# zhiqwang/yolort

Hardware: AMD Instinct MI355X
Metric: images/sec at 640x640 (bs=32) yolov5s (higher is better)
Workload: dtype fp16; 1 GPU; yolov5_darknet_pan_s_r60 fp16 bs=32/GPU 640x640 fixed-size stream (letterbox = identity: the stem reads the planar images) -> backbone+PAN+head+decode+NMS HIP path (BASELINE configs[1]); detections_per_img=300, weights=seeded synthetic (workloads/synth.py, head_gain 0.4), parallelism=dp1 (one shard per rank, slab all-gather), conv_tiles=pinned table yolort_amd/data/tiles_gfx950.json

## Files before the change

yolort_amd/csrc/stem_body1_fused.hip:

```cpp
#include "conv_common.hpp"

namespace ymi {

constexpr int SB_TH = 8, SB_TW = 16;
constexpr int SB_PH = 2 * SB_TH + 1, SB_PW = 2 * SB_TW + 1;
constexpr int SB_NE = SB_TW + 1;
constexpr int SB_PPIX = SB_PH * SB_PW;
constexpr int SB_GROUPS = (SB_PPIX + 31) / 32;
constexpr int SB_IR = 2 * SB_PH + 4, SB_IC = 80;
constexpr int SB_ENTRIES = 3 * SB_IR * (SB_IC / 8);
constexpr int SB_PIECES = (SB_ENTRIES + 63) / 64;
constexpr int SB_SW = SB_PW + 2;
constexpr int SB_SENTRIES = SB_IR * SB_SW;
constexpr int SB_SPIECES = (SB_SENTRIES + 63) / 64;
constexpr int SB_MAX_IMGS = 32;
#ifndef YMI_SB_PK
#define YMI_SB_PK 0
#endif
constexpr bool SB_PK = YMI_SB_PK != 0;

struct SbImgs {
    const uint16_t* img[SB_MAX_IMGS];
};

constexpr int SB_W1 = 0, SB_W2 = 36 * 1024, SB_B2 = 256, SB_PLANAR = SB_SPIECES * 1024, SB_PATCH = ((SB_PPIX + 15) / 16) * 1024;
constexpr int SB_LDS = SB_W1 + SB_W2 + SB_B2 + SB_PLANAR + SB_PATCH;

template <int DT, bool PLANAR>
__global__ __launch_bounds__(512, 1) void stem_body1_fused_kernel(const ConvArgs a1, const ConvArgs a2, const SbImgs pl, int tiles_x, int tiles_y, int ntiles) {
    typedef typename Mfma<DT>::frag frag;
    extern __shared__ __attribute__((aligned(16))) unsigned char sb_sm[];
    frag* w2l = reinterpret_cast<frag*>(sb_sm + SB_W1);
    f32x4* b2l = reinterpret_cast<f32x4*>(sb_sm + SB_W1 + SB_W2);
    uint16_t* planar = reinterpret_cast<uint16_t*>(sb_sm + SB_W1 + SB_W2 + SB_B2);
    unsigned char* patch = sb_sm + SB_W1 + SB_W2 + SB_B2 + SB_PLANAR;

    const int tid = threadIdx.x;
    const int lane = tid & 63;
    const int wave = __builtin_amdgcn_readfirstlane(tid >> 6);
    const int hi = lane >> 5, px = lane & 31;
    const int H = a1.h, W = 2 * a1.w_in;

    {
        for (int f = wave; f < 36; f += 8) {
            const int i = f & 1, ts = f >> 1;
            w2l[f * 64 + lane] = *reinterpret_cast<const frag*>(a2.w + (int64_t)(i * 32 + px) * a2.k_pad + ts * 16 + hi * 8);
        }
        if (tid < 16) {
            const int t = tid >> 3, g = (tid >> 1) & 3, h = tid & 1;
            b2l[tid] = *reinterpret_cast<const f32x4*>(a2.bias + t * 32 + g * 8 + h * 4);
        }
    }
    f32x4 bias1[1][4];
    load_bias<1>(a1, 0, hi, bias1);
    frag wf1[9];
    {
        const uint16_t* wr = a1.w + (int64_t)px * a1.k_pad + 8 * hi;
#pragma unroll
        for (int s = 0; s < 9; ++s) wf1[s] = *reinterpret_cast<const frag*>(wr + 16 * s);
    }

    int e_plane[3], e_row[3], e_col[3];
#pragma unroll
    for (int j = 0; j < 3; ++j) {
        const int e = (wave * 3 + j) * 64 + lane;
        if constexpr (PLANAR) {
            const int ec = e < SB_ENTRIES ? e : SB_ENTRIES - 1;
            const int plane = ec / (SB_IR * (SB_IC / 8));
            const int rem = ec - plane * (SB_IR * (SB_IC / 8));
            const int pr = rem / (SB_IC / 8), seg = rem - pr * (SB_IC / 8);
            e_plane[j] = e < SB_ENTRIES ? plane : -1;
            e_row[j] = pr - 4;
            e_col[j] = 8 * seg - 8;
        } else {
            const int ec = e < SB_SENTRIES ? e : SB_SENTRIES - 1;
            const int pr = ec / SB_SW, sc = ec - pr * SB_SW;
            e_plane[j] = e < SB_SENTRIES ? 0 : -1;
            e_row[j] = pr - 4;
            e_col[j] = sc - 2;
        }
    }
    auto tile_origin = [&](int idx, int& img, int& oy0, int& ox0) {
        int t = xcd_remap(idx, ntiles);
        const int tx = t % tiles_x;
        t /= tiles_x;
        const int ty = t % tiles_y;
        img = t / tiles_y;
        oy0 = ty * SB_TH;
        ox0 = tx * SB_TW;
    };
    auto issue_planar = [&](int idx) {
        int img, oy0, ox0;
        tile_origin(idx, img, oy0, ox0);
        if constexpr (PLANAR) {
            const uint16_t* base = pl.img[img];
#pragma unroll
            for (int j = 0; j < 3; ++j) {
                const int pi = wave * 3 + j;
                if (pi < SB_PIECES) {
                    const int iy = 4 * oy0 + e_row[j], ix = 4 * ox0 + e_col[j];
                    const bool ok = (e_plane[j] >= 0) && ((unsigned)iy < (unsigned)H) && ((unsigned)ix < (unsigned)W);
                    const uint16_t* src = ok ? base + ((int64_t)e_plane[j] * H + iy) * W + ix : a1.zeros;
                    glds16(src, planar + pi * 512);
                }
            }
        } else {
#pragma unroll
            for (int j = 0; j < 3; ++j) {
                const int pi = wave * 3 + j;
                if (pi < SB_SPIECES) {
                    const int iy = 4 * oy0 + e_row[j], isp = 2 * ox0 + e_col[j];
                    const bool ok = (e_plane[j] >= 0) && ((unsigned)iy < (unsigned)H) && ((unsigned)isp < (unsigned)a1.w_in);
                    const uint16_t* src = ok ? a1.x + ((int64_t)(img * H + iy) * a1.w_in + isp) * a1.x_cs : a1.zeros;
                    glds16(src, planar + pi * 512);
                }
            }
        }
    };

    int s1_off[3], s1_rc[3], s1_dst[3];
#pragma unroll
    for (int j = 0; j < 3; ++j) {
        const int g = wave + 8 * j;
        const int q = g * 32 + px;
        const int qc = q < SB_PPIX ? q : SB_PPIX - 1;
        const int pr = qc / SB_PW, rem = qc - pr * SB_PW;
        const int pc = rem < SB_NE ? 2 * rem : 2 * (rem - SB_NE) + 1;
        s1_rc[j] = q < SB_PPIX ? ((pr << 16) | pc) : -1;
        s1_off[j] = PLANAR ? (2 * pr) * SB_IC + 2 * pc + 4
                           : ((2 * pr) * SB_SW + pc) * 8;
        s1_dst[j] = qc * 64 + ((hi ^ ((qc >> 2) & 3)) * 16);
    }
    const int pg = wave & 3, ct = wave >> 2;
    const int pr_o = (pg * 32 + px) / SB_TW, pc_o = (pg * 32 + px) % SB_TW;
    int ea[9];
#pragma unroll
    for (int t = 0; t < 9; ++t) {
        const int dy = t / 3, dx = t % 3;
        const int col = 2 * pc_o + dx;
        const int slot = (col & 1) ? SB_NE + (col >> 1) : (col >> 1);
        const int q = (2 * pr_o + dy) * SB_PW + slot;
        ea[t] = (q * 32 + ((hi ^ ((q >> 2) & 3)) * 8)) * 2;
    }
    constexpr int PLANE_HALFS = SB_IR * SB_IC;

    int idx = blockIdx.x;
    if (idx < ntiles) issue_planar(idx);
    for (; idx < ntiles; idx += gridDim.x) {
        int img, oy0, ox0;
        tile_origin(idx, img, oy0, ox0);
        asm volatile("s_waitcnt vmcnt(0)" ::: "memory");
        __syncthreads();

#pragma unroll
        for (int j = 0; j < 3; ++j) {
            if (wave + 8 * j < SB_GROUPS) {
                f32x16 acc[1][1];
                init_acc<1, 1>(acc, bias1);
                if constexpr (PLANAR) {
                    uint32_t rr[9], gg[9], bb[9];
#pragma unroll
                    for (int s = 0; s < 9; ++s) {
                        const int tap0 = 2 * s, tap1 = 2 * s + 1;
                        const int o0 = (tap0 / 3) * SB_IC + 2 * (tap0 % 3), o1 = (tap1 / 3) * SB_IC + 2 * (tap1 % 3);
                        const uint16_t* p0 = planar + s1_off[j] + (hi ? o1 : o0);
                        rr[s] = *reinterpret_cast<const uint32_t*>(p0);
                        gg[s] = *reinterpret_cast<const uint32_t*>(p0 + PLANE_HALFS);
                        bb[s] = *reinterpret_cast<const uint32_t*>(p0 + 2 * PLANE_HALFS);
                    }
                    __builtin_amdgcn_sched_barrier(0);
#pragma unroll
                    for (int s = 0; s < 9; ++s) {
                        const uint32_t r = rr[s], g = gg[s], b = bb[s];
                        u32x4 q;
                        q[0] = (r & 0xffffu) | (g << 16);
                        q[1] = b & 0xffffu;
                        q[2] = (r >> 16) | (g & 0xffff0000u);
                        q[3] = b >> 16;
                        frag af;
                        __builtin_memcpy(&af, &q, 16);
                        acc[0][0] = Mfma<DT>::run(wf1[s], af, acc[0][0]);
                    }
                } else {
                    frag af[9];
#pragma unroll
                    for (int s = 0; s < 9; ++s) {
                        const int tap0 = 2 * s, tap1 = 2 * s + 1;
                        const int o0 = ((tap0 / 3) * SB_SW + (tap0 % 3)) * 8, o1 = ((tap1 / 3) * SB_SW + (tap1 % 3)) * 8;
                        af[s] = *reinterpret_cast<const frag*>(planar + s1_off[j] + (hi ? o1 : o0));
                    }
                    __builtin_amdgcn_sched_barrier(0);
#pragma unroll
                    for (int s = 0; s < 9; ++s) acc[0][0] = Mfma<DT>::run(wf1[s], af[s], acc[0][0]);
                }
                const u32x2 norv[4] = {};
                u32x4 o[2];
                silu_pack_subtile<DT, false, true, SB_PK>(acc[0][0], norv, o);
                const int sy = 2 * oy0 - 1 + (s1_rc[j] >> 16), sx = 2 * ox0 - 1 + (s1_rc[j] & 0xffff);
                const bool in = s1_rc[j] >= 0 && ((unsigned)sy < (unsigned)a1.ho) && ((unsigned)sx < (unsigned)a1.wo);
                if (!in) {
                    o[0] = u32x4{0u, 0u, 0u, 0u};
                    o[1] = u32x4{0u, 0u, 0u, 0u};
                }
                if (s1_rc[j] >= 0) {
                    *reinterpret_cast<u32x4*>(patch + s1_dst[j]) = o[0];
                    *reinterpret_cast<u32x4*>(patch + (s1_dst[j] ^ 32)) = o[1];
                }
            }
        }
        __syncthreads();
        if (idx + (int)gridDim.x < ntiles) issue_planar(idx + gridDim.x);

        f32x16 acc2[1][1];
#pragma unroll
        for (int g = 0; g < 4; ++g) {
            const f32x4 b = b2l[(ct * 4 + g) * 2 + hi];
#pragma unroll
            for (int e = 0; e < 4; ++e) acc2[0][0][g * 4 + e] = b[e];
        }
#pragma unroll
        for (int half = 0; half < 2; ++half) {
            frag fa[9], fw[9];
#pragma unroll
            for (int u = 0; u < 9; ++u) {
                const int ts = half * 9 + u;
                fa[u] = *reinterpret_cast<const frag*>(patch + ((ts & 1) ? (ea[ts >> 1] ^ 32) : ea[ts >> 1]));
                fw[u] = w2l[(ts * 2 + ct) * 64 + lane];
            }
            __builtin_amdgcn_sched_barrier(0);
#pragma unroll
            for (int u = 0; u < 9; ++u) acc2[0][0] = Mfma<DT>::run(fw[u], fa[u], acc2[0][0]);
        }
        finish_wave_tile<DT, DT, 1, 1>(a2, acc2, ct * 32, hi, [&](int, int64_t& m, bool& ok) {
            const int oy = oy0 + pr_o, ox = ox0 + pc_o;
            ok = oy < a2.ho && ox < a2.wo;
            m = ((int64_t)img * a2.ho + oy) * a2.wo + ox;
        });
    }
}

template <int DT, bool PLANAR>
static int stem_body1_launch_t(const ConvArgs& s0, const ConvArgs& b0, const void* const* imgs, hipStream_t st) {
    const int tiles_x = cdiv(b0.wo, SB_TW), tiles_y = cdiv(b0.ho, SB_TH);
    auto kfn = stem_body1_fused_kernel<DT, PLANAR>;
    { const int rc_lds = allow_big_lds((const void*)kfn, SB_LDS); if (rc_lds != YMI_OK) return rc_lds; }
    const int per_launch = PLANAR ? SB_MAX_IMGS : b0.n;
    for (int base = 0; base < b0.n; base += per_launch) {
        ConvArgs a1 = s0, a2 = b0;
        const int n = b0.n - base < per_launch ? b0.n - base : per_launch;
        a1.n = a2.n = n;
        SbImgs pl;
        for (int i = 0; i < SB_MAX_IMGS; ++i) pl.img[i] = PLANAR ? (const uint16_t*)imgs[base + (i < n ? i : 0)] : nullptr;
        a2.y = (void*)((uint16_t*)b0.y + (int64_t)base * b0.ho * b0.wo * b0.y_cs);
        a2.M = n * a2.ho * a2.wo;
        const int ntiles = n * tiles_x * tiles_y;
        a2.nblk_m = ntiles;
        a2.nblk_n = 1;
        const int resident = 256;
        hipLaunchKernelGGL(kfn, dim3(ntiles < resident ? ntiles : resident), dim3(512), SB_LDS, st, a1, a2, pl, tiles_x, tiles_y, ntiles);
    }
    return check_launch("stem_body1_fused_kernel");
}

static int stem_body1_check(const ConvArgs& a1, const ConvArgs& a2, const char* who) {
    YMI_REQUIRE(a1.cin == 8 && a1.kh == 6 && a1.kw == 3 && a1.sh == 2 && a1.sw == 1 && a1.ph == 2 && a1.pw == 1 && a1.k_pad >= 144 && a1.cout == 32 && a1.cout_pad >= 32 &&
                    a1.zeros != nullptr && a1.split == 0 && a1.res == nullptr && a1.act == YMI_ACT_SILU && a1.chain_w == nullptr && a1.up2 == 0,
                "%s: the first descriptor must be the 32-channel stem in its 6x3 s(2,1) p(2,1) super-pixel form (SiLU, no residual / split / chain)", who);
    YMI_REQUIRE(a2.kh == 3 && a2.kw == 3 && a2.sh == 2 && a2.sw == 2 && a2.ph == 1 && a2.pw == 1 && a2.cin == 32 && a2.k_pad == 288 && a2.cout == 64 && a2.cout_pad >= 64 &&
                    a2.up2 == 0 && a2.chain_w == nullptr && a2.split == 0 && a2.res == nullptr && a2.act == YMI_ACT_SILU,
                "%s: the second descriptor must be Conv(32, 64, k=3, s=2, p=1) with SiLU (no residual / split / chain)", who);
    YMI_REQUIRE(a2.n == a1.n && a2.h == a1.ho && a2.w_in == a1.wo && a2.ho == (a2.h - 1) / 2 + 1 && a2.wo == (a2.w_in - 1) / 2 + 1,
                "%s: the second convolution must read the first one's output (%dx%d), got %dx%d", who, a1.ho, a1.wo, a2.h, a2.w_in);
    YMI_REQUIRE(((int64_t)a2.M + 1) * a2.y_cs < ((int64_t)1 << 31), "%s: output tensor too large for 32-bit offsets", who);
    return YMI_OK;
}

int stem_body1_planar_launch(const ConvArgs& a1, const ConvArgs& a2, const void* const* imgs, int dtype, hipStream_t s) {
    { const int rc = stem_body1_check(a1, a2, "ymi_stem_body1_planar"); if (rc != YMI_OK) return rc; }
    YMI_REQUIRE((2 * a1.w_in) % 8 == 0, "ymi_stem_body1_planar: the image width must be a multiple of 8");
    return dtype == YMI_F16 ? stem_body1_launch_t<YMI_F16, true>(a1, a2, imgs, s) : stem_body1_launch_t<YMI_BF16, true>(a1, a2, imgs, s);
}

int stem_body1_launch(const ConvArgs& a1, const ConvArgs& a2, int dtype, hipStream_t s) {
    { const int rc = stem_body1_check(a1, a2, "ymi_stem_body1"); if (rc != YMI_OK) return rc; }
    YMI_REQUIRE(a1.x != nullptr && a1.x_cs == 8, "ymi_stem_body1: the stem must read the NHWC4 canvas (8 halves per super-pixel)");
    YMI_REQUIRE((int64_t)a1.n * a1.h * a1.w_in * 8 < ((int64_t)1 << 31), "ymi_stem_body1: input canvas too large for 32-bit offsets");
    return dtype == YMI_F16 ? stem_body1_launch_t<YMI_F16, false>(a1, a2, nullptr, s) : stem_body1_launch_t<YMI_BF16, false>(a1, a2, nullptr, s);
}

}
```

Baseline: 27450 images/s.

## Software-pipeline stem+body1 fused kernel with double-buffered LDS and planar pre-conversion

Restructures the fused stem/first-conv kernel so stage 1 of the next tile runs before stage 2 of the current one, using double-buffered super-pixel and patch LDS slots. Planar RGB input now lands in a staging area and is converted once into interleaved super-pixel layout, instead of being repacked inside every MFMA tap. Second-conv weights move from LDS into registers, and the first-conv bias moves to LDS. The aim is to hide global-load latency and cut LDS traffic and barrier stalls, at the cost of more registers and LDS and more complex synchronisation.

```diff
diff --git a/yolort_amd/csrc/stem_body1_fused.hip b/yolort_amd/csrc/stem_body1_fused.hip
--- a/yolort_amd/csrc/stem_body1_fused.hip
+++ b/yolort_amd/csrc/stem_body1_fused.hip
@@ -8,8 +8,8 @@
 constexpr int SB_PPIX = SB_PH * SB_PW;
 constexpr int SB_GROUPS = (SB_PPIX + 31) / 32;
 constexpr int SB_IR = 2 * SB_PH + 4, SB_IC = 80;
-constexpr int SB_ENTRIES = 3 * SB_IR * (SB_IC / 8);
-constexpr int SB_PIECES = (SB_ENTRIES + 63) / 64;
+constexpr int SB_UNITS = SB_IR * (SB_IC / 8);
+constexpr int SB_UPW = 48;
 constexpr int SB_SW = SB_PW + 2;
 constexpr int SB_SENTRIES = SB_IR * SB_SW;
 constexpr int SB_SPIECES = (SB_SENTRIES + 63) / 64;
@@ -18,64 +18,85 @@
 #define YMI_SB_PK 0
 #endif
 constexpr bool SB_PK = YMI_SB_PK != 0;
+#ifndef YMI_SB_PIPE
+#define YMI_SB_PIPE 1
+#endif
+constexpr bool SB_PIPE = YMI_SB_PIPE != 0;
 
 struct SbImgs {
     const uint16_t* img[SB_MAX_IMGS];
 };
 
-constexpr int SB_W1 = 0, SB_W2 = 36 * 1024, SB_B2 = 256, SB_PLANAR = SB_SPIECES * 1024, SB_PATCH = ((SB_PPIX + 15) / 16) * 1024;
-constexpr int SB_LDS = SB_W1 + SB_W2 + SB_B2 + SB_PLANAR + SB_PATCH;
+constexpr int SB_B2 = 512, SB_LAND = 8 * 3 * 1024, SB_SPX = SB_SPIECES * 1024, SB_PATCH = ((SB_PPIX + 15) / 16) * 1024;
+constexpr int sb_nslot(bool planar) { return SB_PIPE && planar ? 2 : 1; }
+constexpr int sb_lds(bool planar) { return SB_B2 + SB_LAND + sb_nslot(planar) * (SB_SPX + SB_PATCH); }
+static_assert(sb_lds(true) <= 160 * 1024, "one CU's LDS");
 
 template <int DT, bool PLANAR>
 __global__ __launch_bounds__(512, 1) void stem_body1_fused_kernel(const ConvArgs a1, const ConvArgs a2, const SbImgs pl, int tiles_x, int tiles_y, int ntiles) {
     typedef typename Mfma<DT>::frag frag;
+    constexpr bool PIPE = SB_PIPE && PLANAR;
+    constexpr int SB_NSLOT = sb_nslot(PLANAR);
     extern __shared__ __attribute__((aligned(16))) unsigned char sb_sm[];
-    frag* w2l = reinterpret_cast<frag*>(sb_sm + SB_W1);
-    f32x4* b2l = reinterpret_cast<f32x4*>(sb_sm + SB_W1 + SB_W2);
-    uint16_t* planar = reinterpret_cast<uint16_t*>(sb_sm + SB_W1 + SB_W2 + SB_B2);
-    unsigned char* patch = sb_sm + SB_W1 + SB_W2 + SB_B2 + SB_PLANAR;
+    f32x4* b2l = reinterpret_cast<f32x4*>(sb_sm);
+    f32x4* b1l = reinterpret_cast<f32x4*>(sb_sm + 256);
+    uint16_t* land = reinterpret_cast<uint16_t*>(sb_sm + SB_B2);
+    uint16_t* spx0 = reinterpret_cast<uint16_t*>(sb_sm + SB_B2 + SB_LAND);
+    unsigned char* patch0 = sb_sm + SB_B2 + SB_LAND + SB_NSLOT * SB_SPX;
 
     const int tid = threadIdx.x;
     const int lane = tid & 63;
     const int wave = __builtin_amdgcn_readfirstlane(tid >> 6);
     const int hi = lane >> 5, px = lane & 31;
     const int H = a1.h, W = 2 * a1.w_in;
-
-    {
-        for (int f = wave; f < 36; f += 8) {
-            const int i = f & 1, ts = f >> 1;
-            w2l[f * 64 + lane] = *reinterpret_cast<const frag*>(a2.w + (int64_t)(i * 32 + px) * a2.k_pad + ts * 16 + hi * 8);
-        }
-        if (tid < 16) {
-            const int t = tid >> 3, g = (tid >> 1) & 3, h = tid & 1;
-            b2l[tid] = *reinterpret_cast<const f32x4*>(a2.bias + t * 32 + g * 8 + h * 4);
-        }
-    }
-    f32x4 bias1[1][4];
-    load_bias<1>(a1, 0, hi, bias1);
+    const int pg = wave & 3, ct = wave >> 2;
+
+    if (tid < 16) {
+        const int t = tid >> 3, g = (tid >> 1) & 3, h = tid & 1;
+        b2l[tid] = *reinterpret_cast<const f32x4*>(a2.bias + t * 32 + g * 8 + h * 4);
+    }
+    if (tid >= 64 && tid < 72) {
+        const int g = (tid >> 1) & 3, h = tid & 1;
+        b1l[tid - 64] = *reinterpret_cast<const f32x4*>(a1.bias + g * 8 + h * 4);
+    }
     frag wf1[9];
     {
         const uint16_t* wr = a1.w + (int64_t)px * a1.k_pad + 8 * hi;
 #pragma unroll
         for (int s = 0; s < 9; ++s) wf1[s] = *reinterpret_cast<const frag*>(wr + 16 * s);
     }
-
-    int e_plane[3], e_row[3], e_col[3];
-#pragma unroll
-    for (int j = 0; j < 3; ++j) {
-        const int e = (wave * 3 + j) * 64 + lane;
-        if constexpr (PLANAR) {
-            const int ec = e < SB_ENTRIES ? e : SB_ENTRIES - 1;
-            const int plane = ec / (SB_IR * (SB_IC / 8));
-            const int rem = ec - plane * (SB_IR * (SB_IC / 8));
-            const int pr = rem / (SB_IC / 8), seg = rem - pr * (SB_IC / 8);
-            e_plane[j] = e < SB_ENTRIES ? plane : -1;
+    frag w2r[18];
+    {
+        const uint16_t* wr = a2.w + (int64_t)(ct * 32 + px) * a2.k_pad + 8 * hi;
+#pragma unroll
+        for (int ts = 0; ts < 18; ++ts) w2r[ts] = *reinterpret_cast<const frag*>(wr + 16 * ts);
+    }
+
+    int e_ok[3], e_row[3], e_col[3];
+    int cv_dst = 0;
+    unsigned cv_mask = 0;
+    if constexpr (PLANAR) {
+        const int u = wave * SB_UPW + lane;
+        const bool ok = lane < SB_UPW && u < SB_UNITS;
+        const int uc = ok ? u : 0;
+        const int pr = uc / (SB_IC / 8), seg = uc - pr * (SB_IC / 8);
+#pragma unroll
+        for (int j = 0; j < 3; ++j) {
+            e_ok[j] = ok;
             e_row[j] = pr - 4;
             e_col[j] = 8 * seg - 8;
-        } else {
+        }
+        cv_dst = (pr * SB_SW + 4 * seg - 2) * 8;
+#pragma unroll
+        for (int k = 0; k < 4; ++k)
+            if (ok && (unsigned)(4 * seg - 2 + k) < (unsigned)SB_SW) cv_mask |= 1u << k;
+    } else {
+#pragma unroll
+        for (int j = 0; j < 3; ++j) {
+            const int e = (wave * 3 + j) * 64 + lane;
             const int ec = e < SB_SENTRIES ? e : SB_SENTRIES - 1;
             const int pr = ec / SB_SW, sc = ec - pr * SB_SW;
-            e_plane[j] = e < SB_SENTRIES ? 0 : -1;
+            e_ok[j] = e < SB_SENTRIES;
             e_row[j] = pr - 4;
             e_col[j] = sc - 2;
         }
@@ -89,20 +110,17 @@
         oy0 = ty * SB_TH;
         ox0 = tx * SB_TW;
     };
-    auto issue_planar = [&](int idx) {
+    auto issue_dma = [&](int idx, uint16_t* spx) {
         int img, oy0, ox0;
         tile_origin(idx, img, oy0, ox0);
         if constexpr (PLANAR) {
             const uint16_t* base = pl.img[img];
 #pragma unroll
             for (int j = 0; j < 3; ++j) {
-                const int pi = wave * 3 + j;
-                if (pi < SB_PIECES) {
-                    const int iy = 4 * oy0 + e_row[j], ix = 4 * ox0 + e_col[j];
-                    const bool ok = (e_plane[j] >= 0) && ((unsigned)iy < (unsigned)H) && ((unsigned)ix < (unsigned)W);
-                    const uint16_t* src = ok ? base + ((int64_t)e_plane[j] * H + iy) * W + ix : a1.zeros;
-                    glds16(src, planar + pi * 512);
-                }
+                const int iy = 4 * oy0 + e_row[j], ix = 4 * ox0 + e_col[j];
+                const bool ok = e_ok[j] && ((unsigned)iy < (unsigned)H) && ((unsigned)ix < (unsigned)W);
+                const uint16_t* src = ok ? base + ((int64_t)j * H + iy) * W + ix : a1.zeros;
+                glds16(src, land + (wave * 3 + j) * 512);
             }
         } else {
 #pragma unroll
@@ -110,12 +128,28 @@
                 const int pi = wave * 3 + j;
                 if (pi < SB_SPIECES) {
                     const int iy = 4 * oy0 + e_row[j], isp = 2 * ox0 + e_col[j];
-                    const bool ok = (e_plane[j] >= 0) && ((unsigned)iy < (unsigned)H) && ((unsigned)isp < (unsigned)a1.w_in);
+                    const bool ok = e_ok[j] && ((unsigned)iy < (unsigned)H) && ((unsigned)isp < (unsigned)a1.w_in);
                     const uint16_t* src = ok ? a1.x + ((int64_t)(img * H + iy) * a1.w_in + isp) * a1.x_cs : a1.zeros;
-                    glds16(src, planar + pi * 512);
-                }
-            }
-        }
+                    glds16(src, spx + pi * 512);
+                }
+            }
+        }
+    };
+    auto convert = [&](uint16_t* spx) {
+        asm volatile("s_waitcnt vmcnt(0)" ::: "memory");
+        const u32x4 r = *reinterpret_cast<const u32x4*>(land + (wave * 3 + 0) * 512 + lane * 8);
+        const u32x4 g = *reinterpret_cast<const u32x4*>(land + (wave * 3 + 1) * 512 + lane * 8);
+        const u32x4 b = *reinterpret_cast<const u32x4*>(land + (wave * 3 + 2) * 512 + lane * 8);
+#pragma unroll
+        for (int k = 0; k < 4; ++k) {
+            u32x4 q;
+            q[0] = (r[k] & 0xffffu) | (g[k] << 16);
+            q[1] = b[k] & 0xffffu;
+            q[2] = (r[k] >> 16) | (g[k] & 0xffff0000u);
+            q[3] = b[k] >> 16;
+            if (cv_mask & (1u << k)) *reinterpret_cast<u32x4*>(spx + cv_dst + 8 * k) = q;
+        }
+        asm volatile("s_waitcnt lgkmcnt(0)" ::: "memory");
     };
 
     int s1_off[3], s1_rc[3], s1_dst[3];
@@ -127,11 +161,9 @@
         const int pr = qc / SB_PW, rem = qc - pr * SB_PW;
         const int pc = rem < SB_NE ? 2 * rem : 2 * (rem - SB_NE) + 1;
         s1_rc[j] = q < SB_PPIX ? ((pr << 16) | pc) : -1;
-        s1_off[j] = PLANAR ? (2 * pr) * SB_IC + 2 * pc + 4
-                           : ((2 * pr) * SB_SW + pc) * 8;
+        s1_off[j] = ((2 * pr) * SB_SW + pc) * 8;
         s1_dst[j] = qc * 64 + ((hi ^ ((qc >> 2) & 3)) * 16);
     }
-    const int pg = wave & 3, ct = wave >> 2;
     const int pr_o = (pg * 32 + px) / SB_TW, pc_o = (pg * 32 + px) % SB_TW;
     int ea[9];
 #pragma unroll
@@ -142,57 +174,30 @@
         const int q = (2 * pr_o + dy) * SB_PW + slot;
         ea[t] = (q * 32 + ((hi ^ ((q >> 2) & 3)) * 8)) * 2;
     }
-    constexpr int PLANE_HALFS = SB_IR * SB_IC;
-
-    int idx = blockIdx.x;
-    if (idx < ntiles) issue_planar(idx);
-    for (; idx < ntiles; idx += gridDim.x) {
+
+    auto stage1 = [&](int idx, const uint16_t* spx, unsigned char* patch) {
         int img, oy0, ox0;
         tile_origin(idx, img, oy0, ox0);
-        asm volatile("s_waitcnt vmcnt(0)" ::: "memory");
-        __syncthreads();
-
 #pragma unroll
         for (int j = 0; j < 3; ++j) {
             if (wave + 8 * j < SB_GROUPS) {
                 f32x16 acc[1][1];
-                init_acc<1, 1>(acc, bias1);
-                if constexpr (PLANAR) {
-                    uint32_t rr[9], gg[9], bb[9];
-#pragma unroll
-                    for (int s = 0; s < 9; ++s) {
-                        const int tap0 = 2 * s, tap1 = 2 * s + 1;
-                        const int o0 = (tap0 / 3) * SB_IC + 2 * (tap0 % 3), o1 = (tap1 / 3) * SB_IC + 2 * (tap1 % 3);
-                        const uint16_t* p0 = planar + s1_off[j] + (hi ? o1 : o0);
-                        rr[s] = *reinterpret_cast<const uint32_t*>(p0);
-                        gg[s] = *reinterpret_cast<const uint32_t*>(p0 + PLANE_HALFS);
-                        bb[s] = *reinterpret_cast<const uint32_t*>(p0 + 2 * PLANE_HALFS);
-                    }
-                    __builtin_amdgcn_sched_barrier(0);
-#pragma unroll
-                    for (int s = 0; s < 9; ++s) {
-                        const uint32_t r = rr[s], g = gg[s], b = bb[s];
-                        u32x4 q;
-                        q[0] = (r & 0xffffu) | (g << 16);
-                        q[1] = b & 0xffffu;
-                        q[2] = (r >> 16) | (g & 0xffff0000u);
-                        q[3] = b >> 16;
-                        frag af;
-                        __builtin_memcpy(&af, &q, 16);
-                        acc[0][0] = Mfma<DT>::run(wf1[s], af, acc[0][0]);
-                    }
-                } else {
-                    frag af[9];
-#pragma unroll
-                    for (int s = 0; s < 9; ++s) {
-                        const int tap0 = 2 * s, tap1 = 2 * s + 1;
-                        const int o0 = ((tap0 / 3) * SB_SW + (tap0 % 3)) * 8, o1 = ((tap1 / 3) * SB_SW + (tap1 % 3)) * 8;
-                        af[s] = *reinterpret_cast<const frag*>(planar + s1_off[j] + (hi ? o1 : o0));
-                    }
-                    __builtin_amdgcn_sched_barrier(0);
-#pragma unroll
-                    for (int s = 0; s < 9; ++s) acc[0][0] = Mfma<DT>::run(wf1[s], af[s], acc[0][0]);
-                }
+                {
+                    f32x4 bias1[1][4];
+#pragma unroll
+                    for (int g = 0; g < 4; ++g) bias1[0][g] = b1l[g * 2 + hi];
+                    init_acc<1, 1>(acc, bias1);
+                }
+                frag af[9];
+#pragma unroll
+                for (int s = 0; s < 9; ++s) {
+                    const int tap0 = 2 * s, tap1 = 2 * s + 1;
+                    const int o0 = ((tap0 / 3) * SB_SW + (tap0 % 3)) * 8, o1 = ((tap1 / 3) * SB_SW + (tap1 % 3)) * 8;
+                    af[s] = *reinterpret_cast<const frag*>(spx + s1_off[j] + (hi ? o1 : o0));
+                }
+                __builtin_amdgcn_sched_barrier(0);
+#pragma unroll
+                for (int s = 0; s < 9; ++s) acc[0][0] = Mfma<DT>::run(wf1[s], af[s], acc[0][0]);
                 const u32x2 norv[4] = {};
                 u32x4 o[2];
                 silu_pack_subtile<DT, false, true, SB_PK>(acc[0][0], norv, o);
@@ -208,9 +213,10 @@
                 }
             }
         }
-        __syncthreads();
-        if (idx + (int)gridDim.x < ntiles) issue_planar(idx + gridDim.x);
-
+    };
+    auto stage2 = [&](int idx, const unsigned char* patch) {
+        int img, oy0, ox0;
+        tile_origin(idx, img, oy0, ox0);
         f32x16 acc2[1][1];
 #pragma unroll
         for (int g = 0; g < 4; ++g) {
@@ -220,22 +226,95 @@
         }
 #pragma unroll
         for (int half = 0; half < 2; ++half) {
-            frag fa[9], fw[9];
+            frag fa[9];
 #pragma unroll
             for (int u = 0; u < 9; ++u) {
                 const int ts = half * 9 + u;
                 fa[u] = *reinterpret_cast<const frag*>(patch + ((ts & 1) ? (ea[ts >> 1] ^ 32) : ea[ts >> 1]));
-                fw[u] = w2l[(ts * 2 + ct) * 64 + lane];
             }
             __builtin_amdgcn_sched_barrier(0);
 #pragma unroll
-            for (int u = 0; u < 9; ++u) acc2[0][0] = Mfma<DT>::run(fw[u], fa[u], acc2[0][0]);
+            for (int u = 0; u < 9; ++u) acc2[0][0] = Mfma<DT>::run(w2r[half * 9 + u], fa[u], acc2[0][0]);
         }
         finish_wave_tile<DT, DT, 1, 1>(a2, acc2, ct * 32, hi, [&](int, int64_t& m, bool& ok) {
             const int oy = oy0 + pr_o, ox = ox0 + pc_o;
             ok = oy < a2.ho && ox < a2.wo;
             m = ((int64_t)img * a2.ho + oy) * a2.wo + ox;
         });
+    };
+
+    auto lds_barrier = [&]() {
+        asm volatile("s_waitcnt lgkmcnt(0)" ::: "memory");
+        __builtin_amdgcn_s_barrier();
+    };
+    const int G = gridDim.x;
+    int idx = blockIdx.x;
+    if (idx >= ntiles) return;
+    if constexpr (!PIPE) {
+        if constexpr (PLANAR) {
+            issue_dma(idx, spx0);
+            convert(spx0);
+            if (idx + G < ntiles) issue_dma(idx + G, spx0);
+        } else {
+            issue_dma(idx, spx0);
+        }
+        for (; idx < ntiles; idx += G) {
+            if constexpr (!PLANAR) asm volatile("s_waitcnt vmcnt(0)" ::: "memory");
+            lds_barrier();
+            stage1(idx, spx0, patch0);
+            lds_barrier();
+            if (idx + G < ntiles) {
+                if constexpr (PLANAR) {
+                    convert(spx0);
+                    if (idx + 2 * G < ntiles) issue_dma(idx + 2 * G, spx0);
+                } else {
+                    issue_dma(idx + G, spx0);
+                }
+            }
+            stage2(idx, patch0);
+        }
+    } else {
+        issue_dma(idx, spx0);
+        if constexpr (PLANAR) {
+            convert(spx0);
+            if (idx + G < ntiles) issue_dma(idx + G, spx0);
+        } else {
+            asm volatile("s_waitcnt vmcnt(0)" ::: "memory");
+        }
+        lds_barrier();
+        if constexpr (!PLANAR) {
+            if (idx + G < ntiles) issue_dma(idx + G, spx0 + SB_SPX / 2);
+        }
+        stage1(idx, spx0, patch0);
+        if constexpr (PLANAR) {
+            if (idx + G < ntiles) {
+                convert(spx0 + SB_SPX / 2);
+                if (idx + 2 * G < ntiles) issue_dma(idx + 2 * G, spx0);
+            }
+        } else {
+            asm volatile("s_waitcnt vmcnt(0)" ::: "memory");
+        }
+        for (int k = 0; idx < ntiles; idx += G, k ^= 1) {
+            uint16_t* const spx_k = spx0 + k * (SB_SPX / 2);
+            uint16_t* const spx_n = spx0 + (k ^ 1) * (SB_SPX / 2);
+            unsigned char* const patch_k = patch0 + k * SB_PATCH;
+            unsigned char* const patch_n = patch0 + (k ^ 1) * SB_PATCH;
+            lds_barrier();
+            const bool n1 = idx + G < ntiles, n2 = idx + 2 * G < ntiles;
+            if constexpr (!PLANAR) {
+                if (n2) issue_dma(idx + 2 * G, spx_k);
+            }
+            if (n1) stage1(idx + G, spx_n, patch_n);
+            if constexpr (PLANAR) {
+                if (n2) {
+                    convert(spx_k);
+                    if (idx + 3 * G < ntiles) issue_dma(idx + 3 * G, spx0);
+                }
+            } else {
+                asm volatile("s_waitcnt vmcnt(0)" ::: "memory");
+            }
+            stage2(idx, patch_k);
+        }
     }
 }
 
@@ -243,7 +322,7 @@
 static int stem_body1_launch_t(const ConvArgs& s0, const ConvArgs& b0, const void* const* imgs, hipStream_t st) {
     const int tiles_x = cdiv(b0.wo, SB_TW), tiles_y = cdiv(b0.ho, SB_TH);
     auto kfn = stem_body1_fused_kernel<DT, PLANAR>;
-    { const int rc_lds = allow_big_lds((const void*)kfn, SB_LDS); if (rc_lds != YMI_OK) return rc_lds; }
+    { const int rc_lds = allow_big_lds((const void*)kfn, sb_lds(PLANAR)); if (rc_lds != YMI_OK) return rc_lds; }
     const int per_launch = PLANAR ? SB_MAX_IMGS : b0.n;
     for (int base = 0; base < b0.n; base += per_launch) {
         ConvArgs a1 = s0, a2 = b0;
@@ -257,7 +336,7 @@
         a2.nblk_m = ntiles;
         a2.nblk_n = 1;
         const int resident = 256;
-        hipLaunchKernelGGL(kfn, dim3(ntiles < resident ? ntiles : resident), dim3(512), SB_LDS, st, a1, a2, pl, tiles_x, tiles_y, ntiles);
+        hipLaunchKernelGGL(kfn, dim3(ntiles < resident ? ntiles : resident), dim3(512), sb_lds(PLANAR), st, a1, a2, pl, tiles_x, tiles_y, ntiles);
     }
     return check_launch("stem_body1_fused_kernel");
 }
```

Measured after the change: 27480 images/s (median of 2 runs). About the same (+0.1%).
